# christianhbye/21cmVAE

Measured on AMD Instinct MI355X. Metric: emulated signals/sec (batched predict), higher is better.
Workload: dtype f16 (f32 accumulate)

## Files before the change

21cmvae_amd/csrc/fused_fwd.h:

```cpp
#pragma once
#ifndef __HIPCC_RTC__
#include <hip/hip_runtime.h>
#endif

#include <type_traits>
#include <utility>

#include "../../include/v21_types.h"
#include "par_transform.h"

namespace v21 {

typedef float f32x16 __attribute__((ext_vector_type(16)));
typedef float f32x4 __attribute__((ext_vector_type(4)));
typedef _Float16 f16x8 __attribute__((ext_vector_type(8)));
typedef __bf16 bf16x8 __attribute__((ext_vector_type(8)));
typedef unsigned u32x4 __attribute__((ext_vector_type(4)));
typedef short i16x2 __attribute__((ext_vector_type(2)));
typedef float f32x2 __attribute__((ext_vector_type(2)));
typedef _Float16 f16x2 __attribute__((ext_vector_type(2)));
typedef __bf16 bf16x2 __attribute__((ext_vector_type(2)));

constexpr int kFragBytes = 1024;
constexpr int kWaves = 4;
template <class P> constexpr int fused_lds() { return P::RING * P::BLK * kFragBytes; }
#ifdef V21_FUSED_STAMP
template <class P> constexpr int fused_lds_alloc() { return fused_lds<P>() + 16384; }
#else
template <class P> constexpr int fused_lds_alloc() { return fused_lds<P>(); }
#endif

template <int Base, int N, class F>
__device__ __forceinline__ void static_for_chunk(F& f) {
  [&]<int... I>(std::integer_sequence<int, I...>) __attribute__((always_inline)) {
    (f(std::integral_constant<int, Base + I>{}), ...);
  }(std::make_integer_sequence<int, N>{});
}
template <int N, class F>
__device__ __forceinline__ void static_for(F&& f) {
  constexpr int CH = 256;
  if constexpr (N <= CH) {
    static_for_chunk<0, N>(f);
  } else {
    [&]<int... C>(std::integer_sequence<int, C...>) __attribute__((always_inline)) {
      (static_for_chunk<C * CH, (N - C * CH < CH ? N - C * CH : CH)>(f), ...);
    }(std::make_integer_sequence<int, (N + CH - 1) / CH>{});
  }
}

struct FusedArgs {
  const float* x;
  long long ldx;
  float* y;
  long long ldy;
  long long n_rows;
  const unsigned char* stream;
  float out_std;
  float out_mean_scale;
  int in_transform;
  v21_affine_in tin;
  unsigned long long* dbg;
  const float* lnl_d;
  const float* lnl_w;
  long long lnl_ld;
  unsigned lnl_wg0, lnl_wgpd;
};

struct PrecF16 {
  static constexpr int BLK = 24, RING = 4, WPS = 1, DEPTH = 2, WAVES = 4;
  using frag = f16x8;
  using elem = _Float16;
  static constexpr int FPI = 16, EPI = 8, CT = 2;
  static constexpr int WPI = 4;
  static __device__ __forceinline__ unsigned pack2(float a, float b) {
    f32x2 v = {a, b};
    return __builtin_bit_cast(unsigned, __builtin_convertvector(v, f16x2));
  }
  template <bool SWAP> static __device__ __forceinline__ f32x16 mfma(frag w, frag x, f32x16 c) {
    if constexpr (!SWAP) return __builtin_amdgcn_mfma_f32_32x32x16_f16(w, x, c, 0, 0, 0);
    else return __builtin_amdgcn_mfma_f32_32x32x16_f16(x, w, c, 0, 0, 0);
  }
};
struct PrecBF16 {
  static constexpr int BLK = 24, RING = 4, WPS = 1, DEPTH = 2, WAVES = 4;
  using frag = bf16x8;
  using elem = __bf16;
  static constexpr int FPI = 16, EPI = 8, CT = 2;
  static constexpr int WPI = 4;
  static __device__ __forceinline__ unsigned pack2(float a, float b) {
    f32x2 v = {a, b};
    return __builtin_bit_cast(unsigned, __builtin_convertvector(v, bf16x2));
  }
  template <bool SWAP> static __device__ __forceinline__ f32x16 mfma(frag w, frag x, f32x16 c) {
    if constexpr (!SWAP) return __builtin_amdgcn_mfma_f32_32x32x16_bf16(w, x, c, 0, 0, 0);
    else return __builtin_amdgcn_mfma_f32_32x32x16_bf16(x, w, c, 0, 0, 0);
  }
};
struct PrecF32 {
  static constexpr int BLK = 24, RING = 4, WPS = 1, DEPTH = 2, WAVES = 4;
  using frag = f32x4;
  using elem = float;
  static constexpr int FPI = 8, EPI = 4, CT = 1;
  static constexpr int WPI = 4;
  template <bool SWAP> static __device__ __forceinline__ f32x16 mfma(frag w, frag x, f32x16 c) {
#pragma unroll
    for (int e = 0; e < 4; ++e) {
      if constexpr (!SWAP) c = __builtin_amdgcn_mfma_f32_32x32x2f32(w[e], x[e], c, 0, 0, 0);
      else c = __builtin_amdgcn_mfma_f32_32x32x2f32(x[e], w[e], c, 0, 0, 0);
    }
    return c;
  }
};

#ifdef V21_FUSED_STAMP
struct PrecF16x2 : PrecF16 { static constexpr int CT = 1, BLK = 16, RING = 4, WPS = 2; };
struct PrecBF16x2 : PrecBF16 { static constexpr int CT = 1, BLK = 16, RING = 4, WPS = 2; };
#else
struct PrecF16x2 : PrecF16 { static constexpr int CT = 1, BLK = 16, RING = 5, WPS = 2; };
struct PrecBF16x2 : PrecBF16 { static constexpr int CT = 1, BLK = 16, RING = 5, WPS = 2; };
#endif

struct PrecF16x2sp : PrecF16x2 { static constexpr bool SPREAD_DMA = true; };
struct PrecBF16x2sp : PrecBF16x2 { static constexpr bool SPREAD_DMA = true; };
struct PrecF16x2spClk : PrecF16x2sp { static constexpr bool CLOCK_STAMPS = true; };
struct PrecBF16x2spClk : PrecBF16x2sp { static constexpr bool CLOCK_STAMPS = true; };
struct PrecF32Lnl : PrecF32 { static constexpr bool LNL = true; };
struct PrecF16x2spLnl : PrecF16x2sp { static constexpr bool LNL = true; };
struct PrecBF16x2spLnl : PrecBF16x2sp { static constexpr bool LNL = true; };
template <class P, class = void> struct lnl_of { static constexpr bool value = false; };
template <class P> struct lnl_of<P, std::void_t<decltype(P::LNL)>> { static constexpr bool value = P::LNL; };
template <class P, class = void> struct clk_of { static constexpr bool value = false; };
template <class P> struct clk_of<P, std::void_t<decltype(P::CLOCK_STAMPS)>> { static constexpr bool value = P::CLOCK_STAMPS; };
template <class P, class = void> struct spread_of { static constexpr bool value = false; };
template <class P> struct spread_of<P, std::void_t<decltype(P::SPREAD_DMA)>> { static constexpr bool value = P::SPREAD_DMA; };

template <class Arch, class P> struct Geo {
  using Prec = P;
  static constexpr int L = Arch::L;
  static constexpr int FPI = P::FPI;
  static constexpr int BLK = P::BLK, RING = P::RING, WAVES = P::WAVES;
  static constexpr int IPT = 16 / P::EPI;
  static constexpr int dim(int i) { return Arch::dims[i]; }
  static constexpr int act(int l) { return Arch::act[l]; }
  static constexpr int ks_of(int l) { return (dim(l) + FPI - 1) / FPI; }
  static constexpr int nt_of(int l) { return (dim(l + 1) + 31) / 32; }
  static constexpr int tile_base(int l, int nt) {
    int f = 0;
    for (int i = 0; i < l; ++i) f += nt_of(i) * (ks_of(i) + 1);
    return f + nt * (ks_of(l) + 1);
  }
  static constexpr int total() { return tile_base(L, 0); }
  static constexpr int padded() { return (total() + 7) / 8 * 8; }
  static constexpr int n_blocks() { return (padded() + BLK - 1) / BLK; }
  static constexpr int blk_glds(int b) {
    if (b < 0 || b >= n_blocks()) return 0;
    const int rem = padded() - b * BLK;
    return (rem < BLK ? rem : BLK) / WAVES;
  }
  static constexpr int ks_max() {
    int m = 0;
    for (int l = 0; l < L; ++l) m = ks_of(l) > m ? ks_of(l) : m;
    return m;
  }
  struct Item { int l, nt, ks; };
  static constexpr Item item_at(int F) {
    for (int l = 0; l < L; ++l) {
      const int tl = ks_of(l) + 1, cnt = nt_of(l) * tl;
      if (F < cnt) return Item{l, F / tl, F % tl - 1};
      F -= cnt;
    }
    return Item{-1, -1, -1};
  }
  static constexpr int gtile(int l, int nt) {
    int g = 0;
    for (int i = 0; i < l; ++i) g += nt_of(i);
    return g + nt;
  }
  static constexpr Item tile_at(int g) {
    for (int l = 0; l < L; ++l) {
      if (g < nt_of(l)) return Item{l, g, -1};
      g -= nt_of(l);
    }
    return Item{-1, -1, -1};
  }
  static constexpr int n_tiles() { return gtile(L, 0); }

  static constexpr int spread_limit(int G) {
    const Item t = tile_at(G), n = tile_at(G + 1);
    if (n.l < 0) return 0;
    if (n.l == t.l && t.l == L - 1) return ks_of(n.l) > P::DEPTH ? ks_of(n.l) - P::DEPTH : 0;
    if (n.l == t.l) return ks_of(n.l);
    const int first_use = IPT * (nt_of(t.l) - 1);
    return first_use < ks_of(n.l) ? first_use : ks_of(n.l);
  }
  static constexpr int chunks_per_kstep(int G, int nchunks) {
    const int lim = spread_limit(G);
    return lim <= 0 ? nchunks : (nchunks + lim - 1) / lim;
  }
  static constexpr int stores_before_step(int S, int CT, int D) {
    int s = 0;
    const int l = L - 1, nch = CT * 8;
    for (int nt = 0; nt + 1 < nt_of(l); ++nt) {
      const int cpk = chunks_per_kstep(gtile(l, nt), nch);
      const int nb = tile_base(l, nt + 1);
      for (int c = 0; c < nch; ++c)
        if (nb + 1 + c / cpk + D < S) s += 2;
    }
    return s;
  }
};

template <int N> __device__ __forceinline__ void wait_vmcnt_barrier() {
  static_assert(N >= 0 && N <= 63, "vmcnt is 6 bits");
  asm volatile("s_waitcnt vmcnt(%0)\n\ts_barrier" ::"n"(N) : "memory");
}

__device__ __forceinline__ void glds16(const unsigned char* sbase, unsigned voff, unsigned lds_dst) {
  asm volatile("s_mov_b32 m0, %2\n\ts_nop 0\n\tglobal_load_lds_dwordx4 %0, %1"
               :
               : "v"(voff), "s"(sbase), "s"(lds_dst)
               : "memory");
}
__device__ __forceinline__ unsigned lds_addr(const void* p) {
  return (unsigned)(unsigned long long)(const __attribute__((address_space(3))) void*)p;
}

template <class G, int B>
__device__ __forceinline__ void issue_block(const unsigned char* gstream, unsigned char* smem,
                                            int wave, int lane) {
  if constexpr (B >= 0 && B < G::n_blocks()) {
    constexpr int NG = G::blk_glds(B);
    const unsigned char* g = gstream + (size_t)B * G::BLK * kFragBytes;
    const unsigned voff = wave * kFragBytes + lane * 16;
    const unsigned s = lds_addr(smem) + (B % G::RING) * G::BLK * kFragBytes + wave * kFragBytes;
    static_for<NG>([&](auto i) __attribute__((always_inline)) {
      constexpr int I = decltype(i)::value;
      glds16(g + I * G::WAVES * kFragBytes, voff, s + I * G::WAVES * kFragBytes);
    });
  }
}

template <class G, int B, int I>
__device__ __forceinline__ void issue_piece(const unsigned char* gstream, unsigned char* smem,
                                            int wave, int lane) {
  if constexpr (B >= 0 && B < G::n_blocks()) {
    if constexpr (I < G::blk_glds(B)) {
      const unsigned char* g = gstream + (size_t)B * G::BLK * kFragBytes + I * G::WAVES * kFragBytes;
      const unsigned voff = wave * kFragBytes + lane * 16;
      const unsigned s = lds_addr(smem) + (B % G::RING) * G::BLK * kFragBytes + wave * kFragBytes +
                         I * G::WAVES * kFragBytes;
      glds16(g, voff, s);
    }
  }
}

template <class G, int CT, int D, int S, bool SPREAD>
__device__ __forceinline__ void ring_boundary(const unsigned char* gstream, unsigned char* smem,
                                              int wave, int lane, unsigned long long* g_dbg = nullptr) {
  constexpr int kBlkFrags = G::BLK, kRing = G::RING;
  if constexpr (S % kBlkFrags == 0 && S < G::padded()) {
    constexpr int B = S / kBlkFrags;
    constexpr int last_issued = (B + kRing - 3 > kRing - 1) ? B + kRing - 3 : kRing - 1;
    constexpr int GA = [] {
      int s = 0;
      for (int i = B + 1; i <= last_issued; ++i) s += G::blk_glds(i);
      return s;
    }();
    constexpr int S_issue = (B < kRing) ? 0 : (B - kRing + 2 + (SPREAD ? 1 : 0)) * kBlkFrags;
    constexpr int SA = lnl_of<typename G::Prec>::value ? 0 : G::stores_before_step(S, CT, D) - G::stores_before_step(S_issue, CT, D);
    constexpr int N = (GA + SA) > 63 ? 63 : (GA + SA);
#ifdef V21_FUSED_STAMP
    { unsigned long long t; asm volatile("s_memtime %0\n\ts_waitcnt lgkmcnt(0)" : "=s"(t)::"memory");
      ((unsigned long long*)(smem + G::RING * G::BLK * kFragBytes))[wave * 512 + 2 * B] = t; }
#endif
    wait_vmcnt_barrier<N>();
#ifdef V21_FUSED_STAMP
    { unsigned long long t; asm volatile("s_memtime %0\n\ts_waitcnt lgkmcnt(0)" : "=s"(t)::"memory");
      ((unsigned long long*)(smem + G::RING * G::BLK * kFragBytes))[wave * 512 + 2 * B + 1] = t; }
#endif
    if constexpr (B >= 2 && !SPREAD) issue_block<G, B + kRing - 2>(gstream, smem, wave, lane);
  }
}

template <class G, int F> __device__ __forceinline__ const unsigned char* frag_ptr(const unsigned char* smem, int lane) {
  constexpr int B = F / G::BLK;
  return smem + ((B % G::RING) * G::BLK + (F % G::BLK)) * kFragBytes + lane * 16;
}

template <class Arch, class P>
__global__ void __launch_bounds__(64 * P::WAVES, P::WPS) fused_fwd(const FusedArgs a) {
  constexpr int kWaves = P::WAVES;
  constexpr int kBlkFrags = P::BLK, kRing = P::RING, kFusedLds = fused_lds<P>();
  (void)kFusedLds;
  extern __shared__ __attribute__((aligned(16))) unsigned char smem[];
  using G = Geo<Arch, P>;
  using frag = typename P::frag;
  using Item = typename G::Item;
  constexpr int L = G::L, CT = P::CT, EPI = P::EPI, FPI = P::FPI, IPT = G::IPT;
  constexpr int KSM = G::ks_max();
#ifndef V21_FUSED_D
#define V21_FUSED_D 2
#endif
#ifndef V21_FUSED_SPREAD
#define V21_FUSED_SPREAD 0
#endif
  constexpr int D = P::DEPTH;
  constexpr bool SPREAD = (V21_FUSED_SPREAD != 0) || spread_of<P>::value;
  constexpr int TOTAL = G::total();
  constexpr int NOUT = G::dim(L);
  constexpr int NCH = CT * 8;
  static_assert(G::act(L - 1) == 0, "output layer must be linear");
  static_assert(G::nt_of(L - 1) == 1 || G::ks_of(L - 1) > P::DEPTH, "output layer: too few k-steps per tile for the aux double buffer");
  static_assert(D <= kBlkFrags, "read-ahead must stay within one block");

  const int lane = threadIdx.x & 63;
  const int wave = __builtin_amdgcn_readfirstlane(threadIdx.x >> 6);
  const int r = lane & 31, h = lane >> 5;
  unsigned long long clk_t0 = 0, clk_r0 = 0;
  if constexpr (clk_of<P>::value) {
    asm volatile("s_memtime %0\n\ts_memrealtime %1\n\ts_waitcnt lgkmcnt(0)" : "=s"(clk_t0), "=s"(clk_r0)::"memory");
  }
  const long long wg_row0 = (long long)blockIdx.x * (kWaves * CT * 32);
  const long long row0 = wg_row0 + wave * (CT * 32);

  constexpr bool LNL = lnl_of<P>::value;
  constexpr int NTO = G::nt_of(L - 1), NTL = LNL ? NTO : 1;
  float lnl_x[NTL];
  unsigned lnl_live = 0;
  float lnl_d = 0.f, lnl_w = 0.f;
  f32x16 lnl_acc;
  static_assert(!LNL || (CT == 1 && NTO <= 32), "ln L variant: one column tile per wave, at most 32 output tiles");
  auto lnl_lane = [&]() __attribute__((always_inline)) {
    return (int)__builtin_amdgcn_mbcnt_hi(~0u, __builtin_amdgcn_mbcnt_lo(~0u, 0u));
  };
  auto lnl_pair = [&](float x, float& d, float& w) __attribute__((always_inline)) {
    const unsigned u = __builtin_bit_cast(unsigned, x);
    const auto p2 = __builtin_amdgcn_permlane32_swap(u, u, false, false);
    d = __builtin_bit_cast(float, (unsigned)p2[0]);
    w = __builtin_bit_cast(float, (unsigned)p2[1]);
  };
  auto lnl_load = [&]() __attribute__((always_inline)) {
    const int ln = lnl_lane(), lr = ln & 31;
    const unsigned drow = (a.lnl_wg0 + blockIdx.x) / a.lnl_wgpd;
    const float* src = (ln >> 5) ? a.lnl_w : a.lnl_d + (long long)drow * a.lnl_ld;
    static_for<NTO>([&](auto nt_) __attribute__((always_inline)) {
      constexpr int nt = decltype(nt_)::value;
      float v = 0.f;
      if (32 * nt + 31 < NOUT || 32 * nt + lr < NOUT) v = src[32 * nt + lr];
      lnl_x[nt] = v;
    });
  };
  auto lnl_pin = [&]() __attribute__((always_inline)) {
    static_for<NTO>([&](auto nt_) __attribute__((always_inline)) {
      constexpr int nt = decltype(nt_)::value;
      asm volatile("" : "+v"(lnl_x[nt]));
      float d, w;
      lnl_pair(lnl_x[nt], d, w);
      lnl_live |= (w != 0.f ? 1u : 0u) << nt;
    });
#pragma unroll
    for (int i = 0; i < 16; ++i) lnl_acc[i] = 0.f;
  };
  constexpr int LNL_S_LOAD = G::tile_base(L - 1, 0);
  constexpr int LNL_C_PIN = G::tile_base(L - 1, 0) + 1;

  unsigned bufA[CT][KSM][4], bufB[CT][KSM][4];

  {
    constexpr int K0 = G::dim(0);
    static_for<CT>([&](auto ct_) __attribute__((always_inline)) {
      constexpr int ct = decltype(ct_)::value;
      const long long row = row0 + ct * 32 + r;
      const bool ok = row < a.n_rows;
      const float* xr = a.x + (ok ? row : 0) * a.ldx;
      static_for<G::ks_of(0)>([&](auto ks_) __attribute__((always_inline)) {
        constexpr int ks = decltype(ks_)::value;
        float v[EPI];
        static_for<EPI>([&](auto e_) __attribute__((always_inline)) {
          constexpr int e = decltype(e_)::value;
          constexpr int f0 = FPI * ks + 8 * (e >> 2) + (e & 3);
          constexpr int f1 = f0 + 4;
          float t = 0.f;
          if constexpr (f0 < K0) {
            const bool valid = ok && (h == 0 || f1 < K0);
            if (valid) {
              t = xr[f0 + 4 * h];
              if (a.in_transform) {
                constexpr int g1 = f1 < 8 ? f1 : 7;
                constexpr int g0 = f0 < 8 ? f0 : 7;
                const double zf = h ? a.tin.zero_floor[g1] : a.tin.zero_floor[g0];
                const int lm = h ? a.tin.log_mask[g1] : a.tin.log_mask[g0];
                const double lo = h ? a.tin.lo[g1] : a.tin.lo[g0];
                const double sp = h ? a.tin.span[g1] : a.tin.span[g0];
                t = par_transform_f32(t, lm, zf, lo, sp);
              }
            }
          }
          v[e] = t;
        });
#pragma unroll
        for (int wd = 0; wd < 4; ++wd) {
          if constexpr (EPI == 8) bufA[ct][ks][wd] = P::pack2(v[2 * wd], v[2 * wd + 1]);
          else bufA[ct][ks][wd] = __builtin_bit_cast(unsigned, v[wd]);
        }
      });
    });
  }

  static_for<kRing>([&](auto b) __attribute__((always_inline)) {
    issue_block<G, decltype(b)::value>(a.stream, smem, wave, lane);
  });

  long long wg_rows = a.n_rows - wg_row0;
  if (wg_rows > kWaves * CT * 32) wg_rows = kWaves * CT * 32;
  if (wg_rows < 0) wg_rows = 0;
  const unsigned out_bytes = (unsigned)(wg_rows * a.ldy * 4);
  __amdgpu_buffer_rsrc_t orsrc =
      __builtin_amdgcn_make_buffer_rsrc((void*)(a.y + wg_row0 * a.ldy), 0, out_bytes, 0x00020000);
  const unsigned ldy_b = (unsigned)a.ldy * 4u;
  const unsigned ovoff = (unsigned)(wave * (CT * 32) + 4 * h) * ldy_b + (unsigned)r * 4u;

  frag q[D + 1];
  f32x16 auxb[2];
  f32x16 acc[2][CT];

  auto epilogue_chunk = [&](auto g_, auto c_) __attribute__((always_inline)) {
    constexpr int GT = decltype(g_)::value;
    constexpr int c = decltype(c_)::value;
    constexpr Item t = G::tile_at(GT);
    constexpr int l = t.l, nt = t.nt;
    constexpr int ct = c / 8, pr = c % 8;
    if constexpr (l < L - 1) {
      constexpr int item = IPT * nt + (2 * pr) / EPI, e0 = (2 * pr) % EPI;
      if constexpr (item < G::ks_of(l + 1)) {
        auto& out = (l & 1) ? bufA : bufB;
        const float x0 = acc[GT & 1][ct][2 * pr], x1 = acc[GT & 1][ct][2 * pr + 1];
        if constexpr (EPI == 8) {
          unsigned w = P::pack2(x0, x1);
          if constexpr (G::act(l) != 0) {
            const i16x2 z = {0, 0};
            w = __builtin_bit_cast(unsigned, __builtin_elementwise_max(__builtin_bit_cast(i16x2, w), z));
          }
          out[ct][item][e0 / 2] = w;
        } else {
          int b0 = __builtin_bit_cast(int, x0), b1 = __builtin_bit_cast(int, x1);
          if constexpr (G::act(l) != 0) { b0 = max(b0, 0); b1 = max(b1, 0); }
          out[ct][item][e0] = (unsigned)b0;
          out[ct][item][e0 + 1] = (unsigned)b1;
        }
      }
    } else {
      const float obias = auxb[GT & 1][0], omean = auxb[GT & 1][1] * a.out_mean_scale;
      unsigned voff = ovoff + (unsigned)(32 * nt) * 4u;
      if (32 * nt + r >= NOUT) voff = 0xFFFFFFF0u;
      if constexpr (LNL && pr == 0) lnl_pair(lnl_x[nt], lnl_d, lnl_w);
#pragma unroll
      for (int u = 0; u < 2; ++u) {
        const int i = 2 * pr + u;
        const unsigned soff = (unsigned)(ct * 32 + (i & 3) + 8 * (i >> 2)) * ldy_b;
        float y;
        if constexpr (EPI == 8) {
          y = __builtin_fmaf(acc[GT & 1][ct][i], a.out_std, __builtin_fmaf(obias, a.out_std, omean));
        } else {
          y = (acc[GT & 1][ct][i] + obias) * a.out_std + omean;
        }
        if constexpr (LNL) {
          const float res = lnl_d - y, wr = lnl_w * res;
          const float sum = __builtin_fmaf(wr, res, lnl_acc[i]);
          lnl_acc[i] = ((lnl_live >> nt) & 1u) ? sum : lnl_acc[i];
        } else {
          __builtin_amdgcn_raw_buffer_store_b32(__builtin_bit_cast(unsigned, y), orsrc, voff, soff, 0);
        }
      }
    }
  };
  auto epilogue_range = [&](auto g_, auto lo_, auto hi_) __attribute__((always_inline)) {
    constexpr int LO = decltype(lo_)::value, HI = decltype(hi_)::value;
    static_for<(HI > LO ? HI - LO : 0)>([&](auto k) __attribute__((always_inline)) {
      epilogue_chunk(g_, std::integral_constant<int, LO + decltype(k)::value>{});
    });
  };
  auto operand = [&](auto& buf, int ct, int ks) __attribute__((always_inline)) {
    const u32x4 wds = {buf[ct][ks][0], buf[ct][ks][1], buf[ct][ks][2], buf[ct][ks][3]};
    return __builtin_bit_cast(frag, wds);
  };

  static_for<TOTAL + D>([&](auto s_) __attribute__((always_inline)) {
    constexpr int S = decltype(s_)::value;
    if constexpr (S < TOTAL) {
      ring_boundary<G, CT, D, S, SPREAD>(a.stream, smem, wave, lane, a.dbg);
      if constexpr (LNL && S == LNL_S_LOAD) lnl_load();
      if constexpr (SPREAD && S / kBlkFrags >= 2) {
        constexpr int Bc = S / kBlkFrags, o = S % kBlkFrags;
#ifndef V21_SP_PHASE
#define V21_SP_PHASE 3
#endif
        if constexpr (o % G::WAVES == V21_SP_PHASE % G::WAVES)
          issue_piece<G, Bc + kRing - 2, o / G::WAVES>(a.stream, smem, wave, lane);
      }
      constexpr Item it = G::item_at(S);
      if constexpr (it.ks >= 0) {
        q[S % (D + 1)] = *(const frag*)frag_ptr<G, S>(smem, lane);
      } else {
        constexpr int GT = G::gtile(it.l, it.nt);
        const unsigned char* aux = frag_ptr<G, S>(smem, 0);
        if constexpr (it.l < L - 1) {
          const f32x4* bp = (const f32x4*)(aux + h * 64);
#pragma unroll
          for (int qd = 0; qd < 4; ++qd) {
            const f32x4 t = bp[qd];
            auxb[GT & 1][4 * qd + 0] = t[0]; auxb[GT & 1][4 * qd + 1] = t[1];
            auxb[GT & 1][4 * qd + 2] = t[2]; auxb[GT & 1][4 * qd + 3] = t[3];
          }
        } else {
          auxb[GT & 1][0] = ((const float*)aux)[r];
          auxb[GT & 1][1] = ((const float*)aux)[32 + r];
        }
      }
    }
    if constexpr (S >= D) {
      constexpr int C = S - D;
      constexpr Item it = G::item_at(C);
      if constexpr (LNL && C == LNL_C_PIN) lnl_pin();
      if constexpr (it.ks >= 0) {
        constexpr int GT = G::gtile(it.l, it.nt);
        constexpr int GP = GT > 0 ? GT - 1 : 0;
        constexpr int CPK = G::chunks_per_kstep(GP, NCH);
        constexpr bool whole_first = (GT > 0) && (G::spread_limit(GP) == 0);
        if constexpr (whole_first && it.ks == 0) {
          epilogue_range(std::integral_constant<int, GP>{}, std::integral_constant<int, 0>{},
                         std::integral_constant<int, NCH>{});
        }
#ifdef V21_FUSED_STAMP
        if constexpr (it.ks == 0) {
          unsigned long long t; asm volatile("s_memtime %0\n\ts_waitcnt lgkmcnt(0)" : "=s"(t)::"memory");
          ((unsigned long long*)(smem + kFusedLds))[wave * 512 + 128 + GT] = t; }
#endif
        auto& in = (it.l & 1) ? bufB : bufA;
        const frag w = q[C % (D + 1)];
#pragma unroll
        for (int ct = 0; ct < CT; ++ct) {
          f32x16 c0;
          if constexpr (it.ks == 0) {
            if constexpr (it.l < L - 1) c0 = auxb[GT & 1];
            else
#pragma unroll
              for (int i = 0; i < 16; ++i) c0[i] = 0.f;
          } else {
            c0 = acc[GT & 1][ct];
          }
          acc[GT & 1][ct] = P::template mfma<(it.l == L - 1)>(w, operand(in, ct, it.ks), c0);
        }
        if constexpr (GT > 0 && !whole_first) {
          constexpr int lo = it.ks * CPK < NCH ? it.ks * CPK : NCH;
          constexpr int hi = (it.ks + 1) * CPK < NCH ? (it.ks + 1) * CPK : NCH;
          epilogue_range(std::integral_constant<int, GP>{}, std::integral_constant<int, lo>{},
                         std::integral_constant<int, hi>{});
        }
      }
    }
  });
  epilogue_range(std::integral_constant<int, G::n_tiles() - 1>{}, std::integral_constant<int, 0>{},
                 std::integral_constant<int, NCH>{});
  if constexpr (LNL) {
    float v[16];
#pragma unroll
    for (int i = 0; i < 16; ++i) v[i] = lnl_acc[i];
    const int ln = lnl_lane(), lr = ln & 31, lh = ln >> 5;
    auto xlane = [&](float x, int m) __attribute__((always_inline)) {
      return __builtin_bit_cast(float, __builtin_amdgcn_ds_bpermute((ln ^ m) << 2, __builtin_bit_cast(int, x)));
    };
    static_for<4>([&](auto s_) __attribute__((always_inline)) {
      constexpr int c = 8 >> decltype(s_)::value, m = 16 >> decltype(s_)::value;
      const bool up = (lr & m) != 0;
#pragma unroll
      for (int j = 0; j < c; ++j) {
        const float keep = up ? v[c + j] : v[j], send = up ? v[j] : v[c + j];
        v[j] = keep + xlane(send, m);
      }
    });
    const float total = v[0] + xlane(v[0], 1);
    const int i = lr >> 1;
    const unsigned row = (unsigned)(wave * 32 + (i & 3) + 8 * (i >> 2) + 4 * lh);
    const unsigned loff = (lr & 1) ? 0xFFFFFFF0u : row * 4u;
    __builtin_amdgcn_raw_buffer_store_b32(__builtin_bit_cast(unsigned, -0.5f * total), orsrc, loff, 0, 0);
  }
  if constexpr (clk_of<P>::value) {
    unsigned long long t1, r1;
    unsigned xcc, hwid;
    asm volatile("s_memtime %0\n\ts_memrealtime %1\n\ts_getreg_b32 %2, hwreg(HW_REG_XCC_ID)\n\ts_getreg_b32 %3, hwreg(HW_REG_HW_ID)\n\ts_waitcnt lgkmcnt(0)"
                 : "=s"(t1), "=s"(r1), "=s"(xcc), "=s"(hwid)::"memory");
    if (a.dbg && wave == 0 && lane == 0) {
      unsigned long long* gd = a.dbg + (size_t)blockIdx.x * 5;
      gd[0] = clk_t0; gd[1] = clk_r0; gd[2] = t1; gd[3] = r1; gd[4] = (unsigned long long)(xcc & 0xF) | ((unsigned long long)hwid << 8);
    }
  }
#ifdef V21_FUSED_STAMP
  if (a.dbg) {
    unsigned long long t; asm volatile("s_memtime %0\n\ts_waitcnt lgkmcnt(0)" : "=s"(t)::"memory");
    unsigned long long* sd = (unsigned long long*)(smem + kFusedLds) + wave * 512;
    sd[127] = t;
    __builtin_amdgcn_s_waitcnt(0xC07F);
    unsigned long long* gd = a.dbg + ((size_t)blockIdx.x * kWaves + wave) * 512;
#pragma unroll
    for (int k = 0; k < 8; ++k) gd[64 * k + lane] = sd[64 * k + lane];
  }
#endif
}

}
```

21cmvae_amd/csrc/par_transform.h:

```cpp
#pragma once
#ifndef __HIPCC_RTC__
#include <hip/hip_runtime.h>
#endif

#include "../../include/v21_types.h"

namespace v21 {
__host__ __device__ __forceinline__ float par_transform_f32(float x, int lm, double zf, double lo, double span) {
  if (zf > 0.0 && x == 0.f) x = (float)zf;
  double t = (double)x;
  if (lm) t = (double)(float)log10(t);
  t -= lo; t /= span; t *= 2.0; t -= 1.0;
  return (float)t;
}
__host__ __device__ __forceinline__ float par_transform_f64(double t, int lm, double zf, double lo, double span) {
  if (zf > 0.0 && t == 0.0) t = zf;
  if (lm) t = log10(t);
  t -= lo; t /= span; t *= 2.0; t -= 1.0;
  return (float)t;
}
}
```

Measured before the change: 1.240 billion.

## Load inputs before ring prologue and use fast double log10 with fallback

Input rows are loaded into registers first. When the first layer has a single K-step, the weight ring prologue is issued right after those loads, so the global input loads overlap the weight streaming, and the parameter transform runs afterwards. The library double log10 in the parameter transform is replaced by an inline polynomial atanh-series log10 in double. It falls back to the library call when rounding to float is ambiguous or the input is not a normal positive float, so results stay correctly rounded at the cost of extra code and register pressure.

```diff
diff --git a/21cmvae_amd/csrc/fused_fwd.h b/21cmvae_amd/csrc/fused_fwd.h
--- a/21cmvae_amd/csrc/fused_fwd.h
+++ b/21cmvae_amd/csrc/fused_fwd.h
@@ -366,34 +366,57 @@
 
   unsigned bufA[CT][KSM][4], bufB[CT][KSM][4];
 
+  auto ring_prologue = [&]() __attribute__((always_inline)) {
+    static_for<kRing>([&](auto b) __attribute__((always_inline)) {
+      issue_block<G, decltype(b)::value>(a.stream, smem, wave, lane);
+    });
+  };
   {
-    constexpr int K0 = G::dim(0);
+    constexpr int K0 = G::dim(0), KS0 = G::ks_of(0);
+    constexpr bool HEAD_EARLY = KS0 == 1;
+    float xv[CT][KS0][EPI];
+    bool okr[CT];
     static_for<CT>([&](auto ct_) __attribute__((always_inline)) {
       constexpr int ct = decltype(ct_)::value;
       const long long row = row0 + ct * 32 + r;
       const bool ok = row < a.n_rows;
+      okr[ct] = ok;
       const float* xr = a.x + (ok ? row : 0) * a.ldx;
-      static_for<G::ks_of(0)>([&](auto ks_) __attribute__((always_inline)) {
+      static_for<KS0 * EPI>([&](auto i_) __attribute__((always_inline)) {
+        constexpr int ks = decltype(i_)::value / EPI, e = decltype(i_)::value % EPI;
+        constexpr int f0 = FPI * ks + 8 * (e >> 2) + (e & 3);
+        constexpr int f1 = f0 + 4;
+        float t = 0.f;
+        if constexpr (f0 < K0) {
+          if (ok && (h == 0 || f1 < K0)) t = xr[f0 + 4 * h];
+          if constexpr (HEAD_EARLY) asm volatile("" : "+v"(t));
+        }
+        xv[ct][ks][e] = t;
+      });
+    });
+    if constexpr (HEAD_EARLY) {
+      ring_prologue();
+      __builtin_amdgcn_sched_barrier(0);
+    }
+    static_for<CT>([&](auto ct_) __attribute__((always_inline)) {
+      constexpr int ct = decltype(ct_)::value;
+      static_for<KS0>([&](auto ks_) __attribute__((always_inline)) {
         constexpr int ks = decltype(ks_)::value;
         float v[EPI];
         static_for<EPI>([&](auto e_) __attribute__((always_inline)) {
           constexpr int e = decltype(e_)::value;
           constexpr int f0 = FPI * ks + 8 * (e >> 2) + (e & 3);
           constexpr int f1 = f0 + 4;
-          float t = 0.f;
+          float t = xv[ct][ks][e];
           if constexpr (f0 < K0) {
-            const bool valid = ok && (h == 0 || f1 < K0);
-            if (valid) {
-              t = xr[f0 + 4 * h];
-              if (a.in_transform) {
-                constexpr int g1 = f1 < 8 ? f1 : 7;
-                constexpr int g0 = f0 < 8 ? f0 : 7;
-                const double zf = h ? a.tin.zero_floor[g1] : a.tin.zero_floor[g0];
-                const int lm = h ? a.tin.log_mask[g1] : a.tin.log_mask[g0];
-                const double lo = h ? a.tin.lo[g1] : a.tin.lo[g0];
-                const double sp = h ? a.tin.span[g1] : a.tin.span[g0];
-                t = par_transform_f32(t, lm, zf, lo, sp);
-              }
+            if (a.in_transform && okr[ct] && (h == 0 || f1 < K0)) {
+              constexpr int g1 = f1 < 8 ? f1 : 7;
+              constexpr int g0 = f0 < 8 ? f0 : 7;
+              const double zf = h ? a.tin.zero_floor[g1] : a.tin.zero_floor[g0];
+              const int lm = h ? a.tin.log_mask[g1] : a.tin.log_mask[g0];
+              const double lo = h ? a.tin.lo[g1] : a.tin.lo[g0];
+              const double sp = h ? a.tin.span[g1] : a.tin.span[g0];
+              t = par_transform_f32(t, lm, zf, lo, sp);
             }
           }
           v[e] = t;
@@ -405,11 +428,8 @@
         }
       });
     });
-  }
-
-  static_for<kRing>([&](auto b) __attribute__((always_inline)) {
-    issue_block<G, decltype(b)::value>(a.stream, smem, wave, lane);
-  });
+    if constexpr (!HEAD_EARLY) ring_prologue();
+  }
 
   long long wg_rows = a.n_rows - wg_row0;
   if (wg_rows > kWaves * CT * 32) wg_rows = kWaves * CT * 32;
diff --git a/21cmvae_amd/csrc/par_transform.h b/21cmvae_amd/csrc/par_transform.h
--- a/21cmvae_amd/csrc/par_transform.h
+++ b/21cmvae_amd/csrc/par_transform.h
@@ -6,12 +6,46 @@
 #include "../../include/v21_types.h"
 
 namespace v21 {
-__host__ __device__ __forceinline__ float par_transform_f32(float x, int lm, double zf, double lo, double span) {
+
+__host__ __device__ __forceinline__ bool par_log10_fast_f32(float x, float* out) {
+  const unsigned u = __builtin_bit_cast(unsigned, x);
+  if (u - 0x00800000u >= 0x7f000000u) return false;
+  const unsigned ix = u - 0x3f3504f3u;
+  const int e = (int)ix >> 23;
+  const float m = __builtin_bit_cast(float, (ix & 0x007fffffu) + 0x3f3504f3u);
+  const double s = ((double)m - 1.0) / ((double)m + 1.0);
+  const double z = s * s;
+  double p = 1.0 / 19.0;
+  p = __builtin_fma(p, z, 1.0 / 17.0);
+  p = __builtin_fma(p, z, 1.0 / 15.0);
+  p = __builtin_fma(p, z, 1.0 / 13.0);
+  p = __builtin_fma(p, z, 1.0 / 11.0);
+  p = __builtin_fma(p, z, 1.0 / 9.0);
+  p = __builtin_fma(p, z, 1.0 / 7.0);
+  p = __builtin_fma(p, z, 1.0 / 5.0);
+  p = __builtin_fma(p, z, 1.0 / 3.0);
+  const double lm = ((s + s) * __builtin_fma(p, z, 1.0)) * 0.43429448190325182765;
+  const double y = __builtin_fma((double)e, 0.30102999566398119521, lm);
+  const float a = (float)__builtin_fma(y, -0x1p-44, y), b = (float)__builtin_fma(y, 0x1p-44, y);
+  *out = a;
+  return a == b;
+}
+__host__ __device__ __forceinline__ float par_log10_f32(float x) {
+  float r;
+  if (par_log10_fast_f32(x, &r)) return r;
+  return (float)log10((double)x);
+}
+__host__ __device__ __forceinline__ float par_floor_log_f32(float x, int lm, double zf) {
   if (zf > 0.0 && x == 0.f) x = (float)zf;
-  double t = (double)x;
-  if (lm) t = (double)(float)log10(t);
+  return lm ? par_log10_f32(x) : x;
+}
+__host__ __device__ __forceinline__ float par_affine_f32(float v, double lo, double span) {
+  double t = (double)v;
   t -= lo; t /= span; t *= 2.0; t -= 1.0;
   return (float)t;
+}
+__host__ __device__ __forceinline__ float par_transform_f32(float x, int lm, double zf, double lo, double span) {
+  return par_affine_f32(par_floor_log_f32(x, lm, zf), lo, span);
 }
 __host__ __device__ __forceinline__ float par_transform_f64(double t, int lm, double zf, double lo, double span) {
   if (zf > 0.0 && t == 0.0) t = zf;
```

Result: no change. 1.246 billion (median of 5 runs) (+0.5%).
